# vmoens/mujoco-torch

Measured on AMD Instinct MI355X. Metric: env-steps/sec, higher is better.
Workload: dtype f64

## Files before the change

mujoco-torch_amd/csrc/mjh_kernels.h:

```cpp
#pragma once
#include <cstring>
#include "mjh_device.h"

template <typename REAL>
struct LdsView {
  REAL* base;
  const LdsOff* off;
#define X(n, c, p) __device__ __forceinline__ REAL* n() const { return base + off->n; }
  MJH_LDS_ARRAYS(X, _)
#undef X
};

#ifndef MJH_NO_NT
#define MJH_NT_STORE(v, p) __builtin_nontemporal_store((v), (p))
#else
#define MJH_NT_STORE(v, p) (*(p) = (v))
#endif
template <typename MM>
inline int lds_carve(const MM& m, int phase_bit, LdsOff& o, int* kv_defer_ok = nullptr) {
  int off = 0;
#define X(n, c, p) o.n = off; if ((p) & phase_bit) off += (((c) + 1) & ~1);
  MJH_LDS_ARRAYS(X, m)
#undef X
  if (phase_bit == PH_CON) {
// ... 988 lines not shown
          rotate(bp, quat, r);
#pragma unroll
          for (int i = 0; i < 3; i++) pos[i] = pos[i] + r[i];
          quat_mul(quat, bq, quat);
        }
        for (int jj = 0; jj < jn; jj++) joint_step(j0 + jj, pos, quat, own);
      }
      }
      if (M.nmocap > 0) {
        const int k = M.body_mocapid[b];
        if (k >= 0) {
          const REAL* mp = in.mocap_pos + (e * M.nmocap + k) * 3;
          const REAL* mq = in.mocap_quat + (e * M.nmocap + k) * 4;
#pragma unroll
          for (int i = 0; i < 3; i++) pos[i] = mp[i];
#pragma unroll
          for (int i = 0; i < 4; i++) quat[i] = mq[i];
          normalize_n<REAL, 4>(quat);
        }
      }
#pragma unroll
      for (int i = 0; i < 3; i++) S.xpos()[3 * b + i] = pos[i];
#pragma unroll
      for (int i = 0; i < 4; i++) S.xquat()[4 * b + i] = quat[i];
      if (M.lds_diet) {
        REAL xm[9], xim[9];
        quat_to_mat(quat, xm);
        local_to_global(pos, quat, M.body_ipos + 3 * b, M.body_iquat + 4 * b, S.xipos() + 3 * b, xim);
        if (out.xmat) {
#pragma unroll
          for (int i = 0; i < 9; i++) MJH_NT_STORE(xm[i], &out.xmat[(e * M.nbody + b) * 9 + i]);
        }
        if (out.ximat) {
#pragma unroll
          for (int i = 0; i < 9; i++) MJH_NT_STORE(xim[i], &out.ximat[(e * M.nbody + b) * 9 + i]);
        }
      } else {
      quat_to_mat(quat, S.xmat() + 9 * b);
      local_to_global(pos, quat, M.body_ipos + 3 * b, M.body_iquat + 4 * b, S.xipos() + 3 * b, S.ximat() + 9 * b);
      }
    }
    wave_sync();
    STAMP(2);
    REAL cam_com[3] = {0, 0, 0};
    if (with_cams && l < M.ncam && in.subtree_com) {
      const int mode = M.cam_mode[l], tgt = M.cam_targetbodyid[l];
      const int sb = mode == CAM_TRACKCOM ? M.cam_bodyid[l] : ((mode == CAM_TARGETBODYCOM && tgt >= 0) ? tgt : -1);
      if (sb >= 0) {
#pragma unroll
        for (int i = 0; i < 3; i++) cam_com[i] = in.subtree_com[(e * M.nbody + sb) * 3 + i];
      }
    }
    if (!(DEFER && W > 16 && M.kv_defer)) frame_stores();
    if constexpr (XK) if (com_first) { com_pos<DEFER>(); wave_sync(); }
    for (int j = l; j < M.njnt; j += W) {
      const int t = M.jnt_type[j], qa = M.jnt_qposadr[j];
      if (t == JNT_FREE || t == JNT_BALL) {
        const int o = (t == JNT_FREE) ? qa + 3 : qa;
#pragma unroll
        for (int i = 0; i < 4; i++) S.qpos()[o + i] = S.jquat()[4 * j + i];
      }
    }
    for (int g = l; g < M.ngeom; g += W) {
      const int b = M.geom_bodyid[g];
      REAL p[3], mat[9];
      local_to_global(S.xpos() + 3 * b, S.xquat() + 4 * b, M.geom_pos + 3 * g, M.geom_quat + 4 * g, p, mat);
      if constexpr (KEEPG) if (g == l) {
#pragma unroll
        for (int i = 0; i < 3; i++) ho_g[i] = p[i];
#pragma unroll
        for (int i = 0; i < 9; i++) ho_g[3 + i] = mat[i];
      }
      if (M.nt_all) {
        if (out.geom_xpos) for (int i = 0; i < 3; i++) MJH_NT_STORE(p[i], &out.geom_xpos[(e * M.ngeom + g) * 3 + i]);
        if (out.geom_xmat) for (int i = 0; i < 9; i++) MJH_NT_STORE(mat[i], &out.geom_xmat[(e * M.ngeom + g) * 9 + i]);
      } else {
      if (out.geom_xpos) for (int i = 0; i < 3; i++) out.geom_xpos[(e * M.ngeom + g) * 3 + i] = p[i];
      if (out.geom_xmat) for (int i = 0; i < 9; i++) out.geom_xmat[(e * M.ngeom + g) * 9 + i] = mat[i];
      }
    }
    {
      if (out.site_xpos || out.site_xmat)
      for (int s = l; s < M.nsite; s += W) {
        const int b = M.site_bodyid[s];
        REAL p[3], mat[9];
        local_to_global(S.xpos() + 3 * b, S.xquat() + 4 * b, M.site_pos + 3 * s, M.site_quat + 4 * s, p, mat);
        if (out.site_xpos) for (int i = 0; i < 3; i++) out.site_xpos[(e * M.nsite + s) * 3 + i] = p[i];
        if (out.site_xmat) for (int i = 0; i < 9; i++) out.site_xmat[(e * M.nsite + s) * 9 + i] = mat[i];
      }
      if (with_cams) {
        for (int c = l; c < M.ncam; c += W) {
          const int b = M.cam_bodyid[c], mode = M.cam_mode[c], tgt = M.cam_targetbodyid[c];
          REAL cp[3], cm[9];
          local_to_global(S.xpos() + 3 * b, S.xquat() + 4 * b, M.cam_pos + 3 * c, M.cam_quat + 4 * c, cp, cm);
          if (mode == CAM_TRACK) {
            for (int i = 0; i < 3; i++) cp[i] = S.xpos()[3 * b + i] + M.cam_pos0[3 * c + i];
            for (int i = 0; i < 9; i++) cm[i] = M.cam_mat0[9 * c + i];
          } else if (mode == CAM_TRACKCOM) {
            REAL r[3];
            rotate(M.cam_pos + 3 * c, S.xquat() + 4 * b, r);
            for (int i = 0; i < 3; i++) cp[i] = (c == l ? cam_com[i] : (in.subtree_com ? in.subtree_com[(e * M.nbody + b) * 3 + i] : (REAL)0)) + r[i];
          } else if ((mode == CAM_TARGETBODY || mode == CAM_TARGETBODYCOM) && tgt >= 0) {
            REAL tp[3];
            for (int i = 0; i < 3; i++)
              tp[i] = (mode == CAM_TARGETBODY) ? S.xpos()[3 * tgt + i] : (c == l ? cam_com[i] : (in.subtree_com ? in.subtree_com[(e * M.nbody + tgt) * 3 + i] : (REAL)0));
            REAL f[3] = {tp[0] - cp[0], tp[1] - cp[1], tp[2] - cp[2]};
            normalize_n<REAL, 3>(f);
            REAL up_hint[3] = {0, 0, 1}, right[3], up[3];
            cross3(f, up_hint, right);
            normalize_n<REAL, 3>(right);
            cross3(right, f, up);
            for (int i = 0; i < 3; i++) { cm[3 * i + 0] = right[i]; cm[3 * i + 1] = up[i]; cm[3 * i + 2] = -f[i]; }
          }
          if (out.cam_xpos) for (int i = 0; i < 3; i++) out.cam_xpos[(e * M.ncam + c) * 3 + i] = cp[i];
          if (out.cam_xmat) for (int i = 0; i < 9; i++) out.cam_xmat[(e * M.ncam + c) * 9 + i] = cm[i];
        }
        for (int q = l; q < M.nlight; q += W) {
          const int b = M.light_bodyid[q];
          REAL r[3], dir[3];
          rotate(M.light_pos + 3 * q, S.xquat() + 4 * b, r);
          rotate(M.light_dir + 3 * q, S.xquat() + 4 * b, dir);
          if (out.light_xpos) for (int i = 0; i < 3; i++) out.light_xpos[(e * M.nlight + q) * 3 + i] = S.xpos()[3 * b + i] + r[i];
          if (out.light_xdir) for (int i = 0; i < 3; i++) out.light_xdir[(e * M.nlight + q) * 3 + i] = dir[i];
        }
      }
    }
    wave_sync();
    STAMP(3);
    put(out.qpos, S.qpos(), M.nq);
    STAMP(4);
  }

  template <bool DEFER = false>
  __device__ __forceinline__ void com_pos() {
    const int l = lane_here();
    const int nb = M.nbody;
    REAL* term = S.cinert();
    for (int w = l; w < nb * 4; w += W) {
      const int b = w >> 2, k = w & 3;
      const REAL mass = M.body_mass[b];
      term[w] = (k < 3) ? S.xipos()[3 * b + k] * mass : mass;
    }
    wave_sync();
    for (int w = l; w < nb * 4; w += W) {
      const int b = w >> 2, k = w & 3;
      const int end = M.body_subtree_end[b];
      REAL acc = 0;
      for (int d = end - 1; d >= b; d--) acc += term[4 * d + k];
      if (k < 3) S.sub_pos()[3 * b + k] = acc; else S.sub_mass()[b] = acc;
    }
    wave_sync();
    for (int w = l; w < nb * 3; w += W) {
      const int b = w / 3;
      const REAL ms = S.sub_mass()[b];
      const REAL den = ms > (REAL)MINVAL_CACHED ? ms : (REAL)MINVAL_CACHED;
      S.subtree_com()[w] = (ms < (REAL)mjMINVAL) ? S.xipos()[w] : S.sub_pos()[w] / den;
    }
    wave_sync();
    STAMP(5);
    for (int b = l; b < nb; b += W) {
      const REAL* rc = S.subtree_com() + 3 * M.body_rootid[b];
      const REAL off[3] = {S.xipos()[3 * b] - rc[0], S.xipos()[3 * b + 1] - rc[1], S.xipos()[3 * b + 2] - rc[2]};
      const REAL mass = M.body_mass[b];
      REAL xi[9];
      if (M.lds_diet) { REAL q_[4]; quat_mul(S.xquat() + 4 * b, M.body_iquat + 4 * b, q_); quat_to_mat(q_, xi); }
      else {
#pragma unroll
        for (int i = 0; i < 9; i++) xi[i] = S.ximat()[9 * b + i];
      }
      const REAL* inr = M.body_inertia + 3 * b;
      const REAL h[3][3] = {{0, -off[2], off[1]}, {off[2], 0, -off[0]}, {-off[1], off[0], 0}};
      REAL I[3][3];
#pragma unroll
      for (int i = 0; i < 3; i++)
#pragma unroll
        for (int j = 0; j < 3; j++) {
          REAL s = 0, hh = 0;
#pragma unroll
          for (int k = 0; k < 3; k++) s += (xi[3 * i + k] * inr[k]) * xi[3 * j + k];
#pragma unroll
          for (int k = 0; k < 3; k++) hh += h[i][k] * h[j][k];
          I[i][j] = s + hh * mass;
        }
      REAL* ci = S.cinert() + 10 * b;
      ci[0] = I[0][0]; ci[1] = I[1][1]; ci[2] = I[2][2]; ci[3] = I[0][1]; ci[4] = I[0][2]; ci[5] = I[1][2];
      ci[6] = off[0] * mass; ci[7] = off[1] * mass; ci[8] = off[2] * mass; ci[9] = mass;
    }
    for (int j = l; j < M.njnt; j += W) {
      const int b = M.jnt_bodyid[j], t = M.jnt_type[j];
      int d = M.jnt_dofadr[j];
      const REAL* rc = S.subtree_com() + 3 * M.body_rootid[b];
      const REAL off[3] = {rc[0] - S.xanchor()[3 * j], rc[1] - S.xanchor()[3 * j + 1], rc[2] - S.xanchor()[3 * j + 2]};
      if (t == JNT_FREE || t == JNT_BALL) {
        if (t == JNT_FREE) {
          for (int r = 0; r < 3; r++) for (int k = 0; k < 6; k++) S.cdof()[6 * (d + r) + k] = (k == 3 + r) ? (REAL)1 : (REAL)0;
          d += 3;
        }
        REAL xmb[9];
        if (M.lds_diet) quat_to_mat(S.xquat() + 4 * b, xmb);
        else {
#pragma unroll
          for (int i = 0; i < 9; i++) xmb[i] = S.xmat()[9 * b + i];
        }
#pragma unroll
        for (int r = 0; r < 3; r++) {
          const REAL a[3] = {xmb[r], xmb[3 + r], xmb[6 + r]};
          REAL c[3];
          cross3(a, off, c);
          for (int k = 0; k < 3; k++) { S.cdof()[6 * (d + r) + k] = a[k]; S.cdof()[6 * (d + r) + 3 + k] = c[k]; }
        }
      } else if (t == JNT_HINGE) {
        REAL c[3];
        cross3(S.xaxis() + 3 * j, off, c);
        for (int k = 0; k < 3; k++) { S.cdof()[6 * d + k] = S.xaxis()[3 * j + k]; S.cdof()[6 * d + 3 + k] = c[k]; }
      } else {
        for (int k = 0; k < 3; k++) { S.cdof()[6 * d + k] = 0; S.cdof()[6 * d + 3 + k] = S.xaxis()[3 * j + k]; }
      }
    }
    wave_sync();
    STAMP(6);
    if (!(DEFER && W > 16 && M.kv_defer)) com_stores();
    STAMP(7);
  }

  template <bool FUSED = false, int MAXN = (W == 16 ? 16 : 32)>
  __device__ __forceinline__ void crb_factor() {
    const int l = lane_here();
    const int nb = M.nbody, nv = M.nv;
    STAMP0();
    if (!FUSED) {
      REAL* const dst[2] = {S.cinert(), S.cdof()};
      const REAL* const src[2] = {out.cinert, out.cdof};
      const int cnt[2] = {10 * nb, 6 * nv};
      multi_load<W, 2, 3>(dst, src, cnt, e);
    }
    wave_sync();
    STAMP(11);
    for (int w = l; w < nb * 10; w += W) {
      const int b = w / 10, k = w - 10 * b;
      REAL acc = 0;
      if (b > 0) {
        const int end = M.body_subtree_end[b];
        for (int d = end - 1; d >= b; d--) acc += S.cinert()[10 * d + k];
      }
      S.crb()[w] = acc;
    }
    wave_sync();
    STAMP(12);
    for (int d = l; d < nv; d += W) inert_mul(S.crb() + 10 * M.dof_bodyid[d], S.cdof() + 6 * d, S.crb_cdof() + 6 * d);
    wave_sync();
    STAMP(13);
    for (int w = l; w < (nv * (nv + 1)) / 2; w += W) S.qMp()[w] = 0;
    wave_sync();
    for (int w = l; w < M.nqmpair; w += W) {
      const int pk = M.qm_pair[w], i = pk >> 8, j = pk & 0xff;
      REAL s = 0;
#pragma unroll
      for (int k = 0; k < 6; k++) s += S.crb_cdof()[6 * i + k] * S.cdof()[6 * j + k];
      if (i == j) s = s + M.dof_armature[i];
      S.qMp()[tri_at<true>(i, j, nv)] = s;
    }
    wave_sync();
    if (M.has_ten_armature) {
      for (int w = l; w < (nv * (nv + 1)) / 2; w += W) S.qMp()[w] = S.qMp()[w] + M.ten_JTAJ[w];
      wave_sync();
    }
    if (out.qM) {
      REAL* gM = out.qM + e * nv * nv;
      for (int w = l; w < nv * nv; w += W) {
        int i, j;
        split_index(w, nv, M.inv_nv, i, j);
        const int hi = i > j ? i : j, lo = i > j ? j : i;
        gM[w] = S.qMp()[(hi * (hi + 1)) / 2 + lo];
      }
    }
    STAMP(14);
    putnt(out.crb, S.crb(), 10 * nb);
    wave_sync();
    STAMP(15);
    chol_factor<W, REAL, MAXN, true>(S.qMp(), S.qLD(), nv);
    STAMP(16);
    put(out.qLD, S.qLD(), nv * nv);
    STAMP(17);
  }

  __device__ __forceinline__ static void plane_sphere_(const REAL* n, const REAL* ppos, const REAL* spos, REAL r, REAL& dist, REAL* pos) {
    const REAL d[3] = {spos[0] - ppos[0], spos[1] - ppos[1], spos[2] - ppos[2]};
    dist = dot3(d, n) - r;
#pragma unroll
    for (int i = 0; i < 3; i++) pos[i] = spos[i] - n[i] * (r + (REAL)0.5 * dist);
  }
  __device__ __forceinline__ static void sphere_sphere_(const REAL* p1, REAL r1, const REAL* p2, REAL r2, REAL& dist, REAL* pos, REAL* n) {
#pragma unroll
    for (int i = 0; i < 3; i++) n[i] = p2[i] - p1[i];
    REAL d = normalize_n<REAL, 3>(n);
    if (d == 0) { n[0] = 1; n[1] = 0; n[2] = 0; }
    d = d - (r1 + r2);
#pragma unroll
    for (int i = 0; i < 3; i++) pos[i] = p1[i] + n[i] * (r1 + d * (REAL)0.5);
    dist = d;
  }
  __device__ __forceinline__ static void closest_segment_point(const REAL* a, const REAL* b, const REAL* pt, REAL* o) {
    const REAL ab[3] = {b[0] - a[0], b[1] - a[1], b[2] - a[2]};
    const REAL pa[3] = {pt[0] - a[0], pt[1] - a[1], pt[2] - a[2]};
    REAL t = dot3(pa, ab) / (dot3(ab, ab) + (REAL)1e-6);
    t = t < 0 ? (REAL)0 : (t > 1 ? (REAL)1 : t);
#pragma unroll
    for (int i = 0; i < 3; i++) o[i] = a[i] + t * ab[i];
  }
  __device__ __forceinline__ static void closest_segment_to_segment(const REAL* a0, const REAL* a1, const REAL* b0, const REAL* b1, REAL* best_a, REAL* best_b) {
    REAL dir_a[3], dir_b[3];
#pragma unroll
    for (int i = 0; i < 3; i++) { dir_a[i] = a1[i] - a0[i]; dir_b[i] = b1[i] - b0[i]; }
    const REAL len_a = normalize_n<REAL, 3>(dir_a), len_b = normalize_n<REAL, 3>(dir_b);
    const REAL hla = len_a * (REAL)0.5, hlb = len_b * (REAL)0.5;
    REAL a_mid[3], b_mid[3], trans[3];
#pragma unroll
    for (int i = 0; i < 3; i++) { a_mid[i] = a0[i] + dir_a[i] * hla; b_mid[i] = b0[i] + dir_b[i] * hlb; trans[i] = a_mid[i] - b_mid[i]; }
    const REAL dadb = dot3(dir_a, dir_b), dat = dot3(dir_a, trans), dbt = dot3(dir_b, trans);
    const REAL denom = 1 - dadb * dadb;
    const REAL ota = (-dat + dadb * dbt) / (denom + (REAL)1e-6);
// ... 698 lines not shown
      }
    }
    if (stage_ad) {
      wave_sync();
      put(out.efc_aref, ad_stage, nefc); put(out.efc_D, ad_stage + nefc, nefc);
    }
    STAMP(26);
    if (FRIC) put(out.efc_J, S.efc_J(), nefc * nv);
    else if (out.efc_J) {
      rebind();
      REAL* gJ = out.efc_J + e * nefc * nv;
      if (nl <= W) {
        const int mycol = l < nl ? M.lim_dof[M.nf + l] : -1;
        for (int w = l; w - l < nl * nv; w += W) {
          int r, d;
          split_index(w < nl * nv ? w : 0, nv, M.inv_nv, r, d);
          const int col = __shfl(mycol, (int)(lane_id() & ~(W - 1)) + r, MJH_WAVE);
          if (w < nl * nv) gJ[w] = (d == col) ? S.efc_jl()[r] : (REAL)0;
        }
      } else
      for (int w = l; w < nl * nv; w += W) {
        int r, d;
        split_index(w, nv, M.inv_nv, r, d);
        gJ[w] = (d == M.jnt_dofadr[M.lim_jnt[r]]) ? S.efc_jl()[r] : (REAL)0;
      }
      if (!DIRECT) for (int w = l; w < (nefc - nl) * nv; w += W) gJ[nl * nv + w] = S.efc_J()[w];
    }
    STAMP(27);
    if (out.efc_frictionloss) for (int r = l; r < nefc; r += W) out.efc_frictionloss[e * nefc + r] = (r >= ne && r < ne + nf) ? M.dof_frictionloss[M.fric_dof[r - ne]] : ((r >= ne + nf && r < ne + nfa) ? M.tendon_frictionloss[M.fric_tendon[r - ne - nf]] : (REAL)0);
  }

  __device__ __forceinline__ void dof_sum(int d, int width, REAL* s) {
    const REAL* p = S.cdof_dot() + 6 * d;
#pragma unroll
    for (int k = 0; k < 6; k++) {
      REAL a = p[k];
      if (width == 3) a = (a + p[6 + k]) + p[12 + k];
      s[k] = a;
    }
  }
  __device__ __forceinline__ void cvel_add_joint(int pk, REAL* v) {
    const int t = (pk & 0xff) - 1, d = pk >> 8;
    REAL s[6];
    dof_sum(d, t == JNT_HINGE || t == JNT_SLIDE ? 1 : 3, s);
#pragma unroll
    for (int k = 0; k < 6; k++) v[k] = v[k] + s[k];
    if (t == JNT_FREE) {
      dof_sum(d + 3, 3, s);
#pragma unroll
      for (int k = 0; k < 6; k++) v[k] = v[k] + s[k];
    }
  }

  template <bool FLUID, bool FUSED = false, bool DEFER = false>
  __device__ __forceinline__ void velocity() {
    const int l = lane_here();
    const int nv = M.nv, nb = M.nbody, nu = M.nu;
    if (!FUSED) load_qpos(false);
    load_qvel(); load_act();
    if (!FUSED) {
      row_load<W>(S.cdof(), out.cdof, 6 * nv, e);
      row_load<W>(S.cinert(), out.cinert, 10 * nb, e);
      REAL* const dst[2] = {S.subtree_com(), S.xipos()};
      const REAL* const src[2] = {out.subtree_com, out.xipos};
      const int cnt[2] = {3 * nb, 3 * nb};
      multi_load<W, 2, 2>(dst, src, cnt, e);
    }
    wave_sync();
    STAMP(31);
    if (FLUID && M.ntendon > 0) {
      const int nt = M.ntendon;
      for (int t = l; t < nt; t += W) {
        REAL len = 0, vel = 0;
        for (int q = M.ten_adr[t]; q < M.ten_adr[t + 1]; q++) len += M.ten_coef[q] * S.qpos()[M.ten_qposadr[q]];
        for (int d = 0; d < nv; d++) vel += M.ten_J0[t * nv + d] * S.qvel()[d];
        S.ten_len()[t] = len;
        if (out.ten_length) out.ten_length[e * nt + t] = len;
        if (out.ten_velocity) out.ten_velocity[e * nt + t] = vel;
        const REAL below = M.tendon_lengthspring[2 * t] - len, above = M.tendon_lengthspring[2 * t + 1] - len;
        REAL fs = below > 0 ? M.tendon_stiffness[t] * below : (REAL)0;
        fs = above < 0 ? M.tendon_stiffness[t] * above : fs;
        S.ten_frc()[t] = fs + (-M.tendon_damping[t] * vel);
      }
      row_store<W>(out.ten_J, M.ten_J0, nt * nv, e);
      wave_sync();
    }
    if (!M.act_simple) row_copy_const<W>(out.actuator_moment, M.act_moment, nu * nv, e);
    if (M.act_simple) {
      for (int i = l; i < nu; i += W) {
        const REAL gear = M.act_gear[6 * i];
        S.act_length()[i] = S.qpos()[M.act_qposadr[i]] * gear;
        S.act_velocity()[i] = gear * S.qvel()[M.act_dofadr[i]];
      }
    } else
    for (int i = l; i < nu; i += W) {
      const REAL* gear = M.act_gear + 6 * i;
      const int jt = M.act_jnttype[i], qa = M.act_qposadr[i];
      REAL len = 0;
      if (FLUID && M.act_trntype[i] == 3) {
        len = S.ten_len()[M.act_trnid[i]] * gear[0];
      } else if (jt == JNT_SLIDE || jt == JNT_HINGE) {
        len = S.qpos()[qa] * gear[0];
      } else {
        const bool inparent = M.act_trntype[i] == 1;
        const REAL* qp = S.qpos() + qa + (jt == JNT_FREE ? 3 : 0);
        const REAL qn[4] = {qp[0], qp[1] * (REAL)-1, qp[2] * (REAL)-1, qp[3] * (REAL)-1};
        REAL ga[3] = {gear[0], gear[1], gear[2]};
// ... 290 lines not shown
      for (int b0 = 0; b0 < nb; b0 += W) {
        const int b = b0 + l;
        const bool has = b < nb;
        const int depth = b0 == 0 ? depth0 : (has ? M.body_depth[b] : 0), par = b0 == 0 ? par0 : (has ? M.body_parentid[b] : 0);
        const int d0 = b0 == 0 ? d00 : (has ? M.body_dofadr[b] : 0), nd = b0 == 0 ? nd0 : ((has && depth > 0) ? M.body_dofnum[b] : 0);
        REAL vm[6] = {0, 0, 0, 0, 0, 0};
        if (nd > 0) {
#pragma unroll
          for (int k = 0; k < 6; k++) {
            REAL s = S.cdof_dot()[6 * d0 + k] * S.qvel()[d0];
            for (int r = 1; r < nd; r++) s = s + S.cdof_dot()[6 * (d0 + r) + k] * S.qvel()[d0 + r];
            vm[k] = s;
          }
        }
        wave_sync();
        for (int kk = 0; kk < md; kk++) {
          if (depth == kk + 1) {
#pragma unroll
            for (int k = 0; k < 6; k++) {
              const REAL c = S.cacc()[6 * par + k];
              S.cacc()[6 * b + k] = nd > 0 ? c + vm[k] : c;
            }
          }
          wave_sync();
        }
      }
      for (int b = l; b < nb; b += W) {
        REAL cacc[6], f1[6], f2[6], f3[6];
#pragma unroll
        for (int k = 0; k < 6; k++) cacc[k] = S.cacc()[6 * b + k];
        inert_mul(S.cinert() + 10 * b, cacc, f1);
        inert_mul(S.cinert() + 10 * b, S.cvel() + 6 * b, f2);
        motion_cross_force(S.cvel() + 6 * b, f2, f3);
#pragma unroll
        for (int k = 0; k < 6; k++) S.cacc()[6 * b + k] = f1[k] + f3[k];
      }
    }
    }
    wave_sync();
    STAMP(36);
    if (M.lds_diet) {
      for (int d = l; d < nv; d += W) {
        const int b = M.dof_bodyid[d], end = M.body_subtree_end[b];
        REAL s = 0;
#pragma unroll
        for (int k = 0; k < 6; k++) {
          REAL acc = 0;
          for (int bb = end - 1; bb >= b; bb--) acc += S.cacc()[6 * bb + k];
          s += S.cdof()[6 * d + k] * acc;
        }
        S.qfrc_bias()[d] = s;
      }
    } else {
    for (int w = l; w < nb * 6; w += W) {
      const int b = w / 6, k = w - 6 * b;
      const int end = M.body_subtree_end[b];
      REAL acc = 0;
      for (int d = end - 1; d >= b; d--) acc += S.cacc()[6 * d + k];
      S.cfrc()[w] = acc;
    }
    wave_sync();
    STAMP(37);
    for (int d = l; d < nv; d += W) {
      REAL s = 0;
      const REAL* cf = S.cfrc() + 6 * M.dof_bodyid[d];
#pragma unroll
      for (int k = 0; k < 6; k++) s += S.cdof()[6 * d + k] * cf[k];
      S.qfrc_bias()[d] = s;
    }
    }
    wave_sync();
    STAMP(38);
    STAMP(39);
  }
  template <bool DEFER = false>
  __device__ __forceinline__ void velocity_stores() {
    const int nv = M.nv, nb = M.nbody, nu = M.nu;
    put(out.actuator_length, S.act_length(), nu); put(out.actuator_velocity, S.act_velocity(), nu);
    if (!(DEFER && W > 16 && M.kv_defer)) { put(out.cvel, S.cvel(), 6 * nb); putnt(out.cdof_dot, S.cdof_dot(), 6 * nv); }
    putnt(out.qfrc_passive, S.qfrc_passive(), nv); putnt(out.qfrc_bias, S.qfrc_bias(), nv);
    if (M.act_simple) row_copy_const<W>(out.actuator_moment, M.act_moment, nu * nv, e);
  }

  static __device__ __forceinline__ REAL clamp_min(REAL x, REAL lo) { return x > lo ? x : lo; }
  static __device__ __forceinline__ REAL sq(REAL x) { return x * x; }
  static __device__ __forceinline__ REAL muscle_sigmoid(REAL x) {
    REAL sol = x * x * x * (3 * x * (2 * x - 5) + 10);
    sol = x <= 0 ? (REAL)0 : sol;
    return x >= 1 ? (REAL)1 : sol;
  }
  static __device__ __forceinline__ REAL muscle_dynamics(REAL ctrl, REAL act, const REAL* prm) {
    const REAL ctrlclamp = ctrl < 0 ? (REAL)0 : (ctrl > 1 ? (REAL)1 : ctrl), actclamp = act < 0 ? (REAL)0 : (act > 1 ? (REAL)1 : act);
    const REAL tau_act = prm[0] * ((REAL)0.5 + (REAL)1.5 * actclamp), tau_deact = prm[1] / ((REAL)0.5 + (REAL)1.5 * actclamp), width = prm[2];
    const REAL dctrl = ctrlclamp - act;
    const REAL tau_hard = dctrl > 0 ? tau_act : tau_deact;
    const REAL q = dctrl / (width + (width == 0 ? (REAL)(float)mjMINVAL : (REAL)0));
    const REAL tau_smooth = tau_deact + (tau_act - tau_deact) * muscle_sigmoid(q + (REAL)0.5);
    const REAL tau = width < (REAL)mjMINVAL ? tau_hard : tau_smooth;
    return dctrl / clamp_min(tau, (REAL)mjMINVAL);
  }
  static __device__ __forceinline__ REAL muscle_gain_length(REAL len, REAL lmin, REAL lmax) {
    const REAL a = (REAL)0.5 * (lmin + 1), b = (REAL)0.5 * (1 + lmax);
    const REAL out0 = (REAL)0.5 * sq((len - lmin) / clamp_min(a - lmin, (REAL)mjMINVAL));
    const REAL out1 = 1 - (REAL)0.5 * sq((1 - len) / clamp_min(1 - a, (REAL)mjMINVAL));
    const REAL out2 = 1 - (REAL)0.5 * sq((len - 1) / clamp_min(b - 1, (REAL)mjMINVAL));
    const REAL out3 = (REAL)0.5 * sq((lmax - len) / clamp_min(lmax - b, (REAL)mjMINVAL));
// ... 776 lines not shown
        REAL q[4] = {qpos[qa], qpos[qa + 1], qpos[qa + 2], qpos[qa + 3]}, w[3] = {qvel[da], qvel[da + 1], qvel[da + 2]}, r[4];
        quat_integrate(q, w, dt, r);
        for (int i = 0; i < 4; i++) o[qa + i] = r[i];
      } else {
        o[qa] = qpos[qa] + dt * qvel[da];
      }
    }
  }

  __device__ __forceinline__ void advance_act(const REAL* act0, const REAL* act_dot, REAL* dst) {
    const REAL dt = M.timestep;
    for (int i = lane(); i < M.nu; i += W) {
      const int dyn = M.act_dyntype[i];
      if (dyn == DYN_NONE) continue;
      const int a = M.act_actadr[i];
      REAL act = act0[a];
      if (dyn == DYN_FILTEREXACT) {
        REAL tau = M.act_dynprm[3 * i];
        tau = tau > (REAL)mjMINVAL ? tau : (REAL)mjMINVAL;
        act = act + act_dot[a] * tau * (1 - r_exp<REAL>(-dt / tau));
      } else {
        act = act + act_dot[a] * dt;
      }
      if (M.act_actlimited[i]) {
        const REAL lo = M.act_actrange[2 * i], hi = M.act_actrange[2 * i + 1];
        act = act < lo ? lo : (act > hi ? hi : act);
      }
      if (dst) dst[e * M.na + a] = act;
    }
  }

  __device__ __forceinline__ void advance(const REAL* qpos0, const REAL* qvel0, const REAL* act0, REAL time0, const REAL* act_dot, const REAL* qacc, const REAL* qvel_for_pos) {
    const int l = lane_here();
    const REAL dt = M.timestep;
    const StatePtrs<REAL>& fin = KA.fin;
    advance_act(act0, act_dot, fin.act);
    for (int d = l; d < M.nv; d += W) S.tmp_nv()[d] = qvel0[d] + qacc[d] * dt;
    wave_sync();
    integrate_pos(qpos0, qvel_for_pos ? qvel_for_pos : S.tmp_nv(), dt, S.tmp_nq());
    wave_sync();
    row_store<W>(fin.qpos, S.tmp_nq(), M.nq, e);
    row_store<W>(fin.qvel, S.tmp_nv(), M.nv, e);
    if (l == 0 && fin.time) fin.time[e] = time0 + dt;
  }

  template <bool DEFER = false, bool KEEPG = false, bool XK = KEEPG>
  __device__ __forceinline__ void run_kin() {
    STAMP0();
    load_qpos(true);
    wave_sync();
    STAMP(1);
    const bool com_first = XK && (__builtin_popcount((unsigned)blockIdx.x & (unsigned)KA.xswap_k) & 1) != 0;
    kinematics<DEFER, KEEPG, XK>(KA.rk_stage <= 0, com_first);
    if (!com_first) com_pos<DEFER>();
  }
  __device__ __forceinline__ void run_crb() { crb_factor<false>(); }
  __device__ __forceinline__ void run_con() {
    STAMP0();
    if (M.ncon > 0) collision<0, false, true>();
    if (KA.stages & 0x78) make_constraint();
    if (M.ncon > 0 && !(FRIC && M.topk) && !consts_done_) contact_const_stores();
  }
  template <int NMAX>
  __device__ __forceinline__ void sol2_prefetch(Sol2Pre<REAL, NMAX>& P) {
    const int l = lane_here();
    const int nq = M.nq, nv = M.nv, na = M.na;
    const bool dof = l < nv;
    P.f = (dof && out.qfrc_smooth) ? out.qfrc_smooth[e * nv + l] : (REAL)0;
    {
      const REAL* gL = out.qLD + e * nv * nv;
#pragma unroll
      for (int k = 0; k < NMAX; k++) P.T.t[k] = (dof && k < nv) ? (k <= l ? gL[l * nv + k] : gL[k * nv + l]) : (REAL)0;
    }
    P.T.inv = 0;
    const REAL* gq = KA.cur.qpos + e * nq;
#pragma unroll
    for (int j = 0; j < 2; j++) P.qp[j] = l + W * j < nq ? gq[l + W * j] : (REAL)0;
    P.ac = 0; P.ad = 0;
    if (l < na) { const REAL* ga = KA.state_from_cur ? KA.cur.act : in.act; P.ac = ga ? ga[e * na + l] : (REAL)0; P.ad = out.act_dot ? out.act_dot[e * na + l] : (REAL)0; }
    P.warm = (dof && KA.warm_src && M.nefc > 0) ? KA.warm_src[e * nv + l] : (REAL)0;
  }
  template <int NMAX>
  __device__ __forceinline__ void make_constraint_cs(Sol2Pre<REAL, NMAX>& pre, Sol2Con<REAL>& C) {
    const int l = lane_here();
#if MJH_CS_PF >= 2
    {
      const REAL* gq = KA.cur.qpos + e * M.nq;
#pragma unroll
      for (int j = 0; j < 2; j++) pre.qp[j] = l + W * j < M.nq ? gq[l + W * j] : (REAL)0;
    }
#endif
    const int nv = M.nv, nefc = M.nefc, nl = M.nl, ncon = M.ncon, rows = M.con_rows;
    const bool elliptic = M.cone == CONE_ELLIPTIC;
    if (!KA.state_from_cur && KA.do_step) for (int i = l; i < nv; i += W) S.qvel()[i] = checked(S.qvel()[i], (REAL)0);
    REAL lpos = 0, linvw = 0;
    int lj = 0;
    C.jl = 0; C.ldof = 0;
    if (l < nl) {
      lj = M.lim_jnt[l];
      C.ldof = M.jnt_dofadr[lj];
    }
    {
      const int qa = l < nl ? M.jnt_qposadr[lj] : 0;
      const int srcl = (int)(lane_id() & ~(W - 1)) + (qa & (W - 1));
      const REAL q0 = __shfl(pre.qp[0], srcl, MJH_WAVE), q1 = __shfl(pre.qp[1], srcl, MJH_WAVE);
      const REAL q = qa < W ? q0 : q1;
      if (l < nl) {
// ... 105 lines not shown
    }
    STAMP(26);
  }
  __device__ __forceinline__ void cs_deferred_stores(const Sol2Con<REAL>& C) {
    const int l = lane_here();
    const int nv = M.nv, nefc = M.nefc, nl = M.nl, nd = nefc - nl, rows = M.con_rows;
    rebind();
    if (out.efc_J) {
      REAL* gJ = out.efc_J + e * nefc * nv;
      const bool dof = l < nv;
      for (int r = 0; r < nl; r++) {
        const int col = sub_read<W>(C.ldof, r);
        const REAL v = sub_read<W>(C.jl, r);
        if (dof) MJH_NT_STORE((l == col) ? v : (REAL)0, &gJ[r * nv + l]);
      }
      const int* slot = reinterpret_cast<const int*>(S.i_crow_act());
      const REAL* Jc = S.efc_Jc();
      REAL* gC = gJ + nl * nv;
      for (int c = 0; c < M.ncon; c++) {
        const int at = slot[c];
        for (int sub = 0; sub < rows; sub += 4) {
          REAL v[4];
#pragma unroll
          for (int t = 0; t < 4; t++) v[t] = (at >= 0 && sub + t < rows && dof) ? Jc[(at * rows + sub + t) * nv + l] : (REAL)0;
#pragma unroll
          for (int t = 0; t < 4; t++) if (sub + t < rows && dof) MJH_NT_STORE(v[t], &gC[(c * rows + sub + t) * nv + l]);
        }
      }
    }
    if (out.efc_frictionloss) for (int r = l; r < nefc; r += W) MJH_NT_STORE((REAL)0, &out.efc_frictionloss[e * nefc + r]);
    if (M.ncon > 0) contact_const_stores();
  }
  template <int NMAX, int RPL, bool ONE = false, bool HANDOFF = false>
  __device__ __forceinline__ void run_con_sol2() {
    static_assert(W == 32 && !FRIC && !DIRECT, "plain constraint stage, two environments per wavefront");
    Sol2Pre<REAL, NMAX> pre;
    Sol2Con<REAL> con;
    STAMP0();
    collision<NMAX, HANDOFF>(&pre);
#if MJH_CS_PF == 1
    sol2_prefetch<NMAX>(pre);
#endif
    make_constraint_cs<NMAX>(pre, con);
#if MJH_CS_PF == 3
    if (HANDOFF && ho_on_) {
      __builtin_amdgcn_fence(__ATOMIC_RELEASE, "workgroup");
      __builtin_amdgcn_fence(__ATOMIC_ACQUIRE, "workgroup");
    }
    sol2_prefetch<NMAX>(pre);
#endif
    wave_sync();
    run_sol2<NMAX, RPL, false, true, ONE>(&pre, &con);
  }
  template <bool FLUID, bool FUSED = false, bool DEFER = false>
  __device__ __forceinline__ void run_vel() {
    STAMP0();
    velocity<FLUID, FUSED, DEFER>();
    if (KA.stages & 0x60) actuation<FLUID>();
    velocity_stores<DEFER>();
  }

  __device__ __forceinline__ void run_sol() {
    const int l = lane_here();
    const int nq = M.nq, nv = M.nv, na = M.na;
    STAMP0();
    load_factor_and_accelerate((KA.stages & 0x40) != 0);
    if (!(KA.stages & 0x40)) return;
    STAMP(53);
    if (M.nefc == 0) {
      for (int d = l; d < nv; d += W) S.qacc()[d] = S.qacc_smooth()[d];
      wave_sync();
      put(out.qacc, S.qacc(), nv);
    } else {
      solve();
    }
    integrate_tail();
  }

  template <int NMAX>
  __device__ __forceinline__ void load_damping_rows(TriPack<REAL, NMAX>& Hh) {
    const int l = lane_here();
    const int nv = M.nv;
    const REAL* gM = out.qM + e * nv * nv;
#pragma unroll
    for (int k = 0; k < NMAX; k++) Hh.t[k] = (l < nv && k <= l) ? gM[k * nv + l] : (REAL)0;
  }
  template <int NLO = 0, int NHI = (1 << 30)>
  __device__ __forceinline__ void integrate_tail() {
    const int l = lane_here();
    const int nq = M.nq, nv = M.nv, na = M.na;
    if (!KA.do_step) return;
    rebind();
    const REAL dt = M.timestep;
    const REAL time0 = in.time ? in.time[e] : (REAL)0;
    const int rk = KA.rk_stage;
    if (rk < 0) {
      const REAL* qacc = S.qacc();
      constexpr bool REGSOL = NHI <= 32;
      if (!(M.disableflags & DSBL_EULERDAMP)) {
        if constexpr (REGSOL && NLO > 16) {
          TriPack<REAL, NHI> Hh;
          load_damping_rows<NHI>(Hh);
          const REAL dd = l < nv ? M.timestep * M.dof_damping[l] : (REAL)0;
          const REAL rhs = l < nv ? S.qfrc_smooth()[l] + (M.nefc ? S.qfrc_constraint()[l] : (in.qfrc_constraint ? in.qfrc_constraint[e * nv + l] : (REAL)0)) : (REAL)0;
#pragma unroll
          for (int k = 0; k < NHI; k++) Hh.t[k] = (k == l) ? Hh.t[k] + dd : Hh.t[k];
          chol_pack_big<W, REAL, NHI>(Hh, S.chol_col(), nv);
          const REAL x = tri_solve<W, REAL, NHI>(Hh, rhs, nv);
          if (l < nv) S.s_Mgrad()[l] = x;
          wave_sync();
// ... 924 lines not shown
    }
    return;
  }
  const int64_t blk = blockIdx.x;
  if constexpr (STAGE) {
    const int64_t idx = blk * NSUB + sub;
    const bool consts_early = (K.stage_parts & 1) && (__builtin_popcount((unsigned)blockIdx.x & (unsigned)K.xswap_c) & 1) != 0;
    if (K.stage_parts & 1) {
    if (idx < K.env_count) {
      Env<REAL, 16, false> A(lds, K.env_begin + idx, K.flags);
      if (consts_early && K.M.ncon > 0 && !K.M.topk) A.contact_const_stores();
      A.template run_kin<false, false, true>(); wave_sync();
      if (!((__builtin_popcount((unsigned)blockIdx.x & (((unsigned)K.flags >> 16) & 0xfffu)) & 1) != 0)) { A.template crb_factor<true>(); wave_sync(); A.template run_vel<false, true>(); }
      else { A.template run_vel<false, true>(); wave_sync(); A.template crb_factor<true>(); }
    }
    __builtin_amdgcn_fence(__ATOMIC_RELEASE, "workgroup");
    __builtin_amdgcn_fence(__ATOMIC_ACQUIRE, "workgroup");
    wave_sync();
    }
    {
      const int sub2 = (int)(threadIdx.x >> 5);
      REAL* lds2 = reinterpret_cast<REAL*>(lds_raw) + sub2 * K.lds_reals2;
      for (int p = 0; p < 2; p++) {
        const int64_t i2 = blk * NSUB + 2 * p + sub2;
        if (i2 < K.env_count) {
          Env<REAL, 32, false, true> C(lds2, K.env_begin + i2, K.flags);
          C.S.off = &K.off2;
          C.consts_done_ = consts_early;
          C.run_con();
        }
        wave_sync();
      }
    }
    __builtin_amdgcn_fence(__ATOMIC_RELEASE, "workgroup");
    __builtin_amdgcn_fence(__ATOMIC_ACQUIRE, "workgroup");
    wave_sync();
    if (idx < K.env_count) {
      REAL* lds3 = reinterpret_cast<REAL*>(lds_raw) + sub * K.lds_reals3;
      Env<REAL, 16, false> E(lds3, K.env_begin + idx, K.flags);
      E.S.off = &K.off3;
      E.template run_sol2<NMAX, RPL, NEWTON_ONLY>();
    }
  } else
  {
    const int64_t idx = blk * NSUB + sub;
    if (idx < K.env_count) {
      Env<REAL, W, false> E(lds, K.env_begin + idx, K.flags);
      if constexpr (ALL) {
        const bool swap_cv = (__builtin_popcount((unsigned)blockIdx.x & (((unsigned)K.flags >> 16) & 0xfffu)) & 1) != 0;
        E.template run_kin<false, true>();
        wave_sync();
        REAL h_qv_early = 0;
        if (!swap_cv) {
          E.template crb_factor<true, NMAX>();
          wave_sync();
          E.template run_vel<false, true>();
        } else {
          E.template run_vel<false, true>();
          wave_sync();
          { const int l_ = (int)(threadIdx.x & (W - 1)); h_qv_early = l_ < K.M.nv ? E.S.qvel()[l_] : (REAL)0; }
          wave_sync();
          E.template crb_factor<true, NMAX>();
          wave_sync();
        }
        if (K.M.all_handoff) {
          const int l = (int)(threadIdx.x & (W - 1));
          const int nv6 = 6 * K.M.nv, nb3 = 3 * K.M.nbody, ng = K.M.ngeom;
          REAL h_cd[6], h_sc[3], h_qv;
#pragma unroll
          for (int k = 0; k < 6; k++) h_cd[k] = l + W * k < nv6 ? E.S.cdof()[l + W * k] : (REAL)0;
#pragma unroll
          for (int k = 0; k < 3; k++) h_sc[k] = l + W * k < nb3 ? E.S.subtree_com()[l + W * k] : (REAL)0;
          h_qv = swap_cv ? h_qv_early : (l < K.M.nv ? E.S.qvel()[l] : (REAL)0);
          wave_sync();
          E.S.off = &K.off2;
#pragma unroll
          for (int k = 0; k < 6; k++) if (l + W * k < nv6) E.S.cdof()[l + W * k] = h_cd[k];
#pragma unroll
          for (int k = 0; k < 3; k++) if (l + W * k < nb3) E.S.subtree_com()[l + W * k] = h_sc[k];
          if (l < K.M.nv) E.S.qvel()[l] = h_qv;
          if (l < ng) {
#pragma unroll
            for (int i = 0; i < 3; i++) E.S.geom_xpos()[3 * l + i] = E.ho_g[i];
#pragma unroll
            for (int i = 0; i < 9; i++) E.S.geom_xmat()[9 * l + i] = E.ho_g[3 + i];
          }
          E.ho_on_ = true;
          wave_sync();
        } else {
        __builtin_amdgcn_fence(__ATOMIC_RELEASE, "workgroup");
        __builtin_amdgcn_fence(__ATOMIC_ACQUIRE, "workgroup");
        wave_sync();
        E.S.off = &K.off2;
        }
        E.template run_con_sol2<NMAX, RPL, ONE, true>();
      } else
      if constexpr (CS) E.template run_con_sol2<NMAX, RPL, ONE>();
      else E.template run_sol2<NMAX, RPL, NEWTON_ONLY>();
    }
  }
}

template <typename REAL, int PHASE, int W>
__global__ void __launch_bounds__(phase_threads(PHASE), (phase_waves<REAL, PHASE, W>())) mjh_phase_kernel(KArgs<REAL> args) {
  extern __shared__ __attribute__((aligned(16))) unsigned char lds_raw[];
  const KArgs<REAL>& K = kargs<REAL>();
  constexpr int NSUB = MJH_WAVE / W;
  const int sub = (W == MJH_WAVE) ? 0 : (int)((threadIdx.x & (MJH_WAVE - 1)) / W);
  REAL* lds = reinterpret_cast<REAL*>(lds_raw) + sub * K.lds_reals;
  {
    const int64_t blk = blockIdx.x;
    Env<REAL, W, PHASE == MJH_KERNEL_SOL_GEN || PHASE == MJH_KERNEL_CON_GEN, PHASE == MJH_KERNEL_CON_DIRECT> E(lds, K.env_begin + blk * NSUB + sub, K.flags);
    if (PHASE == MJH_KERNEL_KIN) E.template run_kin<false>();
    else if (PHASE == MJH_KERNEL_CRB) E.run_crb();
    else if (PHASE == MJH_KERNEL_CON || PHASE == MJH_KERNEL_CON_GEN || PHASE == MJH_KERNEL_CON_DIRECT) E.run_con();
// ... 16 lines not shown
```

Measured before the change: 30.53 million.

## Batch model-table loads and chunk subtree sums in com_pos, crb_factor and velocity

```diff
diff --git a/mujoco-torch_amd/csrc/mjh_kernels.h b/mujoco-torch_amd/csrc/mjh_kernels.h
--- a/mujoco-torch_amd/csrc/mjh_kernels.h
+++ b/mujoco-torch_amd/csrc/mjh_kernels.h
@@ -1064,7 +1064,7 @@
       }
     }
     if (!(DEFER && W > 16 && M.kv_defer)) frame_stores();
-    if constexpr (XK) if (com_first) { com_pos<DEFER>(); wave_sync(); }
+    if constexpr (XK) if (com_first) { com_pos<DEFER, KEEPG>(); wave_sync(); }
     for (int j = l; j < M.njnt; j += W) {
       const int t = M.jnt_type[j], qa = M.jnt_qposadr[j];
       if (t == JNT_FREE || t == JNT_BALL) {
@@ -1143,17 +1143,85 @@
     STAMP(4);
   }
 
-  template <bool DEFER = false>
+  template <int NC, int SUB_CH>
+  __device__ __forceinline__ static REAL subtree_sum_chunked(const REAL* src, int b, int end) {
+    REAL acc = 0;
+    for (int d = end - 1; d >= b; d -= SUB_CH) {
+      REAL v[SUB_CH];
+#pragma unroll
+      for (int c = 0; c < SUB_CH; c++) { const int dd = d - c; v[c] = src[NC * (dd > b ? dd : b)]; }
+#pragma unroll
+      for (int c = 0; c < SUB_CH; c++) acc = (d - c >= b) ? acc + v[c] : acc;
+    }
+    return acc;
+  }
+  template <int NC, int MAXT, int SUB_CH, typename SKIP, typename ST>
+  __device__ __forceinline__ void subtree_sums_batched(const REAL* src, int nb, SKIP&& skip, ST&& st) {
+    const int l = lane_here(), n = nb * NC;
+    const int* const ends_tab = M.body_subtree_end;
+    int ends[MAXT];
+#pragma unroll
+    for (int t = 0; t < MAXT; t++) { const int w = l + t * W; ends[t] = w < n ? ends_tab[w / NC] : 0; }
+#pragma unroll
+    for (int t = 0; t < MAXT; t++) {
+      if (t * W >= n) break;
+      const int w = l + t * W;
+      if (w < n) {
+        const int b = w / NC, k = w - NC * b;
+        st(w, b, k, subtree_sum_chunked<NC, SUB_CH>(src + k, b, skip(b) ? b : ends[t]));
+      }
+    }
+    for (int w = l + MAXT * W; w < n; w += W) {
+      const int b = w / NC, k = w - NC * b;
+      st(w, b, k, subtree_sum_chunked<NC, SUB_CH>(src + k, b, skip(b) ? b : ends_tab[b]));
+    }
+  }
+
+  template <bool DEFER = false, bool BATCH = false>
   __device__ __forceinline__ void com_pos() {
     const int l = lane_here();
     const int nb = M.nbody;
     REAL* term = S.cinert();
+    int rid0 = 0, jb0 = 0, jt0 = 0, jd0 = 0, jrid0 = 0;
+    REAL mass0 = 0, inr0[3] = {0, 0, 0};
+    if constexpr (BATCH) {
+      if (l < nb) {
+        rid0 = M.body_rootid[l]; mass0 = M.body_mass[l];
+#pragma unroll
+        for (int i = 0; i < 3; i++) inr0[i] = M.body_inertia[3 * l + i];
+      }
+      if (l < M.njnt) { jb0 = M.jnt_bodyid[l]; jt0 = M.jnt_type[l]; jd0 = M.jnt_dofadr[l]; }
+    }
+    if constexpr (BATCH) {
+      constexpr int MT = 4;
+      const REAL* const mtab = M.body_mass;
+      const REAL* const xip = S.xipos();
+      REAL ms[MT];
+#pragma unroll
+      for (int t = 0; t < MT; t++) ms[t] = l + t * W < nb * 4 ? mtab[(l + t * W) >> 2] : (REAL)0;
+#pragma unroll
+      for (int t = 0; t < MT; t++) {
+        const int w = l + t * W, b = w >> 2, k = w & 3;
+        if (w < nb * 4) term[w] = (k < 3) ? xip[3 * b + k] * ms[t] : ms[t];
+      }
+      for (int w = l + MT * W; w < nb * 4; w += W) {
+        const int b = w >> 2, k = w & 3;
+        const REAL mass = mtab[b];
+        term[w] = (k < 3) ? xip[3 * b + k] * mass : mass;
+      }
+    } else
     for (int w = l; w < nb * 4; w += W) {
       const int b = w >> 2, k = w & 3;
       const REAL mass = M.body_mass[b];
       term[w] = (k < 3) ? S.xipos()[3 * b + k] * mass : mass;
     }
-    wave_sync();
+    if constexpr (BATCH) if (l < M.njnt) jrid0 = M.body_rootid[jb0];
+    wave_sync();
+    if constexpr (BATCH) {
+      REAL* const sp = S.sub_pos();
+      REAL* const sm = S.sub_mass();
+      subtree_sums_batched<4, 4, 1>(term, nb, [](int) { return false; }, [&](int, int b, int k, REAL acc) { if (k < 3) sp[3 * b + k] = acc; else sm[b] = acc; });
+    } else
     for (int w = l; w < nb * 4; w += W) {
       const int b = w >> 2, k = w & 3;
       const int end = M.body_subtree_end[b];
@@ -1171,16 +1239,17 @@
     wave_sync();
     STAMP(5);
     for (int b = l; b < nb; b += W) {
-      const REAL* rc = S.subtree_com() + 3 * M.body_rootid[b];
+      const bool pre = BATCH && b == l;
+      const REAL* rc = S.subtree_com() + 3 * (pre ? rid0 : M.body_rootid[b]);
       const REAL off[3] = {S.xipos()[3 * b] - rc[0], S.xipos()[3 * b + 1] - rc[1], S.xipos()[3 * b + 2] - rc[2]};
-      const REAL mass = M.body_mass[b];
+      const REAL mass = pre ? mass0 : M.body_mass[b];
       REAL xi[9];
       if (M.lds_diet) { REAL q_[4]; quat_mul(S.xquat() + 4 * b, M.body_iquat + 4 * b, q_); quat_to_mat(q_, xi); }
       else {
 #pragma unroll
         for (int i = 0; i < 9; i++) xi[i] = S.ximat()[9 * b + i];
       }
-      const REAL* inr = M.body_inertia + 3 * b;
+      const REAL inr[3] = {pre ? inr0[0] : M.body_inertia[3 * b], pre ? inr0[1] : M.body_inertia[3 * b + 1], pre ? inr0[2] : M.body_inertia[3 * b + 2]};
       const REAL h[3][3] = {{0, -off[2], off[1]}, {off[2], 0, -off[0]}, {-off[1], off[0], 0}};
       REAL I[3][3];
 #pragma unroll
@@ -1199,9 +1268,10 @@
       ci[6] = off[0] * mass; ci[7] = off[1] * mass; ci[8] = off[2] * mass; ci[9] = mass;
     }
     for (int j = l; j < M.njnt; j += W) {
-      const int b = M.jnt_bodyid[j], t = M.jnt_type[j];
-      int d = M.jnt_dofadr[j];
-      const REAL* rc = S.subtree_com() + 3 * M.body_rootid[b];
+      const bool pre = BATCH && j == l;
+      const int b = pre ? jb0 : M.jnt_bodyid[j], t = pre ? jt0 : M.jnt_type[j];
+      int d = pre ? jd0 : M.jnt_dofadr[j];
+      const REAL* rc = S.subtree_com() + 3 * (pre ? jrid0 : M.body_rootid[b]);
       const REAL off[3] = {rc[0] - S.xanchor()[3 * j], rc[1] - S.xanchor()[3 * j + 1], rc[2] - S.xanchor()[3 * j + 2]};
       if (t == JNT_FREE || t == JNT_BALL) {
         if (t == JNT_FREE) {
@@ -1235,7 +1305,7 @@
     STAMP(7);
   }
 
-  template <bool FUSED = false, int MAXN = (W == 16 ? 16 : 32)>
+  template <bool FUSED = false, int MAXN = (W == 16 ? 16 : 32), bool BATCH = false>
   __device__ __forceinline__ void crb_factor() {
     const int l = lane_here();
     const int nb = M.nbody, nv = M.nv;
@@ -1248,6 +1318,10 @@
     }
     wave_sync();
     STAMP(11);
+    if constexpr (BATCH) {
+      REAL* const crb = S.crb();
+      subtree_sums_batched<10, 10, 4>(S.cinert(), nb, [](int b) { return b == 0; }, [&](int w, int, int, REAL acc) { crb[w] = acc; });
+    } else
     for (int w = l; w < nb * 10; w += W) {
       const int b = w / 10, k = w - 10 * b;
       REAL acc = 0;
@@ -1264,6 +1338,39 @@
     STAMP(13);
     for (int w = l; w < (nv * (nv + 1)) / 2; w += W) S.qMp()[w] = 0;
     wave_sync();
+    if constexpr (BATCH) {
+      constexpr int QT = 14;
+      const int np = M.nqmpair;
+      const int* const ptab = M.qm_pair;
+      const REAL* const atab = M.dof_armature;
+      const REAL* const cc = S.crb_cdof();
+      const REAL* const cd = S.cdof();
+      REAL* const qmp = S.qMp();
+      int pk[QT];
+      REAL arm[QT];
+#pragma unroll
+      for (int t = 0; t < QT; t++) pk[t] = l + t * W < np ? ptab[l + t * W] : 0;
+#pragma unroll
+      for (int t = 0; t < QT; t++) arm[t] = (l + t * W < np && (pk[t] >> 8) == (pk[t] & 0xff)) ? atab[pk[t] >> 8] : (REAL)0;
+#pragma unroll
+      for (int t = 0; t < QT; t++) {
+        if (!(t & 1) && t * W >= np) break;
+        const int i = pk[t] >> 8, j = pk[t] & 0xff;
+        REAL s = 0;
+#pragma unroll
+        for (int k = 0; k < 6; k++) s += cc[6 * i + k] * cd[6 * j + k];
+        if (i == j) s = s + arm[t];
+        if (l + t * W < np) qmp[tri_at<true>(i, j, nv)] = s;
+      }
+      for (int w = l + QT * W; w < np; w += W) {
+        const int p = ptab[w], i = p >> 8, j = p & 0xff;
+        REAL s = 0;
+#pragma unroll
+        for (int k = 0; k < 6; k++) s += cc[6 * i + k] * cd[6 * j + k];
+        if (i == j) s = s + atab[i];
+        qmp[tri_at<true>(i, j, nv)] = s;
+      }
+    } else
     for (int w = l; w < M.nqmpair; w += W) {
       const int pk = M.qm_pair[w], i = pk >> 8, j = pk & 0xff;
       REAL s = 0;
@@ -1279,6 +1386,26 @@
     }
     if (out.qM) {
       REAL* gM = out.qM + e * nv * nv;
+      if constexpr (BATCH) {
+        constexpr int ROW_CH = 4;
+        const int nn = nv * nv;
+        const REAL* const qmp = S.qMp();
+        int qW, rW, i, j;
+        split_index(W, nv, M.inv_nv, qW, rW);
+        split_index(l, nv, M.inv_nv, i, j);
+        for (int w0 = l; w0 < nn; w0 += ROW_CH * W) {
+          REAL v[ROW_CH];
+#pragma unroll
+          for (int c = 0; c < ROW_CH; c++) {
+            const int hi = i > j ? i : j, lo = i > j ? j : i;
+            v[c] = qmp[w0 + c * W < nn ? (hi * (hi + 1)) / 2 + lo : 0];
+            i += qW; j += rW;
+            if (j >= nv) { j -= nv; i++; }
+          }
+#pragma unroll
+          for (int c = 0; c < ROW_CH; c++) if (w0 + c * W < nn) gM[w0 + c * W] = v[c];
+        }
+      } else
       for (int w = l; w < nv * nv; w += W) {
         int i, j;
         split_index(w, nv, M.inv_nv, i, j);
@@ -2083,7 +2210,7 @@
     }
   }
 
-  template <bool FLUID, bool FUSED = false, bool DEFER = false>
+  template <bool FLUID, bool FUSED = false, bool DEFER = false, bool BATCH = false>
   __device__ __forceinline__ void velocity() {
     const int l = lane_here();
     const int nv = M.nv, nb = M.nbody, nu = M.nu;
@@ -2480,6 +2607,10 @@
         S.qfrc_bias()[d] = s;
       }
     } else {
+    if constexpr (BATCH) {
+      REAL* const cfrc = S.cfrc();
+      subtree_sums_batched<6, 6, 4>(S.cacc(), nb, [](int) { return false; }, [&](int w, int, int, REAL acc) { cfrc[w] = acc; });
+    } else
     for (int w = l; w < nb * 6; w += W) {
       const int b = w / 6, k = w - 6 * b;
       const int end = M.body_subtree_end[b];
@@ -3362,7 +3493,7 @@
     STAMP(1);
     const bool com_first = XK && (__builtin_popcount((unsigned)blockIdx.x & (unsigned)KA.xswap_k) & 1) != 0;
     kinematics<DEFER, KEEPG, XK>(KA.rk_stage <= 0, com_first);
-    if (!com_first) com_pos<DEFER>();
+    if (!com_first) com_pos<DEFER, KEEPG>();
   }
   __device__ __forceinline__ void run_crb() { crb_factor<false>(); }
   __device__ __forceinline__ void run_con() {
@@ -3574,10 +3705,10 @@
     wave_sync();
     run_sol2<NMAX, RPL, false, true, ONE>(&pre, &con);
   }
-  template <bool FLUID, bool FUSED = false, bool DEFER = false>
+  template <bool FLUID, bool FUSED = false, bool DEFER = false, bool BATCH = false>
   __device__ __forceinline__ void run_vel() {
     STAMP0();
-    velocity<FLUID, FUSED, DEFER>();
+    velocity<FLUID, FUSED, DEFER, BATCH>();
     if (KA.stages & 0x60) actuation<FLUID>();
     velocity_stores<DEFER>();
   }
@@ -4608,15 +4739,15 @@
         wave_sync();
         REAL h_qv_early = 0;
         if (!swap_cv) {
-          E.template crb_factor<true, NMAX>();
+          E.template crb_factor<true, NMAX, true>();
           wave_sync();
-          E.template run_vel<false, true>();
+          E.template run_vel<false, true, false, true>();
         } else {
-          E.template run_vel<false, true>();
+          E.template run_vel<false, true, false, true>();
           wave_sync();
           { const int l_ = (int)(threadIdx.x & (W - 1)); h_qv_early = l_ < K.M.nv ? E.S.qvel()[l_] : (REAL)0; }
           wave_sync();
-          E.template crb_factor<true, NMAX>();
+          E.template crb_factor<true, NMAX, true>();
           wave_sync();
         }
         if (K.M.all_handoff) {
```

Result: faster. 31.07 million, median of 6 (+1.8%).
